# michelebanfi/qLDPC-branched-off

Hardware: AMD Instinct MI355X
Metric: decoded shots/sec, [[144,12,12]] p=0.005 50 BP iters (higher is better)
Workload: dtype f64

## Files before the change

### qldpc-branched-off_amd/csrc/common.h

```cpp
#pragma once
#include <hip/hip_runtime.h>
#include <stdint.h>

#include <algorithm>
#include <cstdarg>
#include <cstdio>
#include <functional>
#include <memory>
#include <mutex>
#include <string>
#include <vector>

#include "../../include/qldpc_hip.h"
#include "stage_layout.h"

#define QLDPC_EXPORT extern "C" __attribute__((visibility("default")))

namespace qldpc {

void set_error(const char *fmt, ...);

#define QLDPC_HIP_TRY(expr)                                                                     \
    do {                                                                                        \
        hipError_t _e = (expr);                                                                 \
// ... 209 lines not shown
    int32_t *d_row_of_slot = nullptr, *d_col_of_slot = nullptr;
    uint8_t *d_deg_of_rslot = nullptr, *d_deg_of_row = nullptr;
    uint16_t *d_deg_of_cslot = nullptr, *d_deg_of_col = nullptr;
    uint16_t *d_ell_col_s = nullptr;
    uint32_t *d_ell_var_s = nullptr;
    int32_t *d_identity = nullptr;
    mutable std::vector<qldpc::DevBuf> owned;
    template <class T> int own(T **view, const std::vector<T> &v) const {
        qldpc::DevBuf b;
        const int rc = qldpc::upload(b, v);
        *view = rc == QLDPC_OK ? b.as<T>() : nullptr;
        if (rc == QLDPC_OK) owned.push_back(std::move(b));
        return rc;
    }
    int32_t *d_regown = nullptr;
    mutable std::mutex mu;
    mutable qldpc::DevBuf ws_msg, ws_qold, ws_vals, ws_misc, ws_queue, ws_list, ws_prior, ws_redo;
    mutable qldpc::DevBuf ws_cs;
    mutable qldpc::DevBuf ws_squeue;
    mutable bool ws_private = false;
    mutable qldpc::StreamHandover ws_hand;
    int ws_acquire(hipStream_t stream) const;
    int ws_release(hipStream_t stream) const;
    mutable std::mutex mu_io;
    mutable qldpc::DevBuf ws_io;
    struct AlphaEntry {
        std::vector<double> host;
        qldpc::PinnedBuf pinned;
        qldpc::DevBuf dev;
        hipEvent_t ready = nullptr;
// ... 15 lines not shown
```

### qldpc-branched-off_amd/csrc/graph.hip

```cpp
#include "common.h"
#include "launchers.h"
#include "regular_plan.h"
#include "regular_own.h"

#include <algorithm>
#include <atomic>
#include <cstring>

namespace qldpc {

static thread_local std::string g_last_error;

void set_error(const char *fmt, ...) {
    char buf[1024];
    va_list ap;
    va_start(ap, fmt);
    vsnprintf(buf, sizeof(buf), fmt, ap);
    va_end(ap);
    g_last_error = buf;
}

int use_device(int device) {
    int count = 0;
    hipError_t e = hipGetDeviceCount(&count);
// ... 291 lines not shown
        }
        std::vector<int32_t> ident(std::max(std::max(m, n), 1));
        for (size_t i = 0; i < ident.size(); i++) ident[i] = (int32_t)i;
        if (rc == QLDPC_OK) rc = g->own(&g->d_row_of_slot, ros);
        if (rc == QLDPC_OK) rc = g->own(&g->d_col_of_slot, cos);
        if (rc == QLDPC_OK) rc = g->own(&g->d_deg_of_rslot, drs);
        if (rc == QLDPC_OK) rc = g->own(&g->d_deg_of_cslot, dcs);
        if (rc == QLDPC_OK) rc = g->own(&g->d_deg_of_row, dr);
        if (rc == QLDPC_OK) rc = g->own(&g->d_deg_of_col, dc);
        if (rc == QLDPC_OK) rc = g->own(&g->d_ell_col_s, ecs);
        if (rc == QLDPC_OK) rc = g->own(&g->d_ell_var_s, evs);
        if (rc == QLDPC_OK) rc = g->own(&g->d_identity, ident);
    }
    if (rc == QLDPC_OK && g->max_row_deg == kRegOwnCdeg && g->max_col_deg == kRegOwnVdeg && n == 2 * m && m <= 1024) {
        std::vector<int32_t> own;
        if (regular_own_assign(m, n, indptr, indices, regular_row_stride(kRegOwnCdeg), own, regular_own_search_choice())) rc = g->own(&g->d_regown, own);
    }
    if (rc != QLDPC_OK) return rc;
    *out = G.release();
    return QLDPC_OK;
}

QLDPC_EXPORT void qldpc_graph_destroy(qldpc_graph *g) {
    if (!g) return;
    (void)hipSetDevice(g->device);
    if (g->wg2_cache) qldpc::wg2_cache_free(g->wg2_cache);
    delete g;
}

QLDPC_EXPORT int qldpc_graph_dims(const qldpc_graph *g, int *m, int *n, int *nnz) {
    QLDPC_REQUIRE(g != nullptr, "graph is NULL");
// ... 6 lines not shown
```

### qldpc-branched-off_amd/csrc/launchers.h

```cpp
#pragma once
#include "common.h"

#include <functional>
#include <vector>

struct qldpc_window_decoder;
struct qldpc_layered_decoder;

namespace qldpc {

struct OsdLaunch;
struct OsdGjArgs;
struct DemTab;
struct SigTab;
struct JudgeSector;
struct EventsSector;

#define QLDPC_FLAG_PUBLIC_MASK 0x0FFFFFFF
#define QLDPC_FLAG_INTERNAL_PRIOR_FINITE 0x40000000
#define QLDPC_FLAG_INTERNAL_PRIOR_LE_CLIP 0x20000000
#define QLDPC_FLAG_INTERNAL_OSD_QUEUE_CLEAN 0x10000000

int minsum_stream_launch(const qldpc_graph *g, int64_t B, const int8_t *d_synd, const double *d_prior, int max_iter,
                         const double *d_alpha, double damping, double clip, int flags, int8_t *d_err, double *d_llr,
// ... 7 lines not shown
int mc_resident_launch(const qldpc_graph *g, int64_t B, const double *d_prior, int max_iter, const double *d_alpha, double clip, int flags,
                       uint64_t seed, int64_t shot_begin, uint32_t thr, int use_osd, const uint64_t *d_Lmask, void *d_cold, hipStream_t stream);
bool regular_supported(const qldpc_graph *g, double clip, int max_iter);
int minsum_regular_launch(const qldpc_graph *g, int64_t B, const int8_t *d_synd, const double *d_prior, int max_iter,
                          const double *d_alpha, double damping, double clip, int flags, bool nanfree, int8_t *d_err, double *d_llr,
                          uint8_t *d_conv, int32_t *d_iter, hipStream_t stream);
int mc_regular_launch(const qldpc_graph *g, int64_t B, const double *d_prior, int max_iter, const double *d_alpha, double clip, int flags,
                      bool nanfree, uint64_t seed, int64_t shot_begin, uint32_t thr, int use_osd, const uint64_t *d_Lmask,
                      void *d_cold, hipStream_t stream, const int32_t *d_shot_list = nullptr, const int32_t *d_shot_count = nullptr);
bool mc_first_table(const qldpc_graph *g, double p0, double alpha0, double clip, int max_iter, unsigned &negbits);
int mc_first_launch(const qldpc_graph *g, int k, const int32_t *d_lptr, const int32_t *d_lidx, int64_t B, uint64_t seed, int64_t shot_begin, uint32_t thr,
                    unsigned negbits, unsigned long long *d_tally, int32_t *d_cont_list, int32_t *d_cont_count, unsigned long long *d_clk, hipStream_t stream);
void mc_first_set_bits(int bits);
void regular_set_list_shots(int s);
void regular_set_own_edges(int v);
int regular_own_search_choice();
void mc_set_big_lanes(int n);
int mc_tail_overlap_choice();
int mc_first_choice();
int mc_regular_fill_cold(void *d_cold, unsigned long long *d_tally, int32_t *d_fail_count, int32_t *d_fail_list, int8_t *f_synd,
                         int8_t *f_err, int8_t *f_hard, double *f_llr, unsigned long long *d_clk);
size_t mc_regular_cold_bytes();
int judge_failed_launch(const qldpc_graph *g, int32_t *d_count, bool reset_counters, int *d_osd_queue, const uint64_t *d_Lmask, const int8_t *f_err, const int8_t *f_synd,
                        const int8_t *f_dec, unsigned long long *d_tally, hipStream_t stream);
bool wave_supported(const qldpc_graph *g, double damping, bool clean);
int wave_kernel_choice();
int minsum_wave_launch(const qldpc_graph *g, int64_t B, const int8_t *d_synd, const double *d_prior, int max_iter, const double *d_alpha,
                       double clip, int flags, int8_t *d_err, double *d_llr, uint8_t *d_conv, int32_t *d_iter, hipStream_t stream);
int mc_wave_launch(const qldpc_graph *g, int64_t B, const double *d_prior, int max_iter, const double *d_alpha, double clip, int flags,
                   uint64_t seed, int64_t shot_begin, uint32_t thr, int use_osd, const uint64_t *d_Lmask, void *d_cold, hipStream_t stream);
// ... 103 lines not shown
```

### qldpc-branched-off_amd/csrc/minsum_regular.hip

```cpp
#include "common.h"
#include "launchers.h"
#include "clocks.h"
#include "mc_common.h"
#include "minsum_common.h"
#include "minsum_f64.h"
#include "regular_plan.h"
#include "regular_own.h"

#include <atomic>
#include <cstdlib>

namespace qldpc {

struct RegArgs {
    int m, n, max_iter, fixed, S, TS;
    const int32_t *indptr, *indices, *colptr, *rowidx, *csc2csr;
    const int32_t *own;
    int64_t B;
    const double *prior, *alpha;
    double damping, clip;
    const int8_t *synd; int8_t *out_err; double *out_llr; uint8_t *out_conv; int32_t *out_iter;
    uint32_t seed_lo, seed_hi, thr; int use_osd;
    int64_t shot_begin;
    const uint64_t *Lmask;
    const int32_t *shot_list, *shot_count;
    const struct RegCold *cold;
    int offV, offE, offL, offI, offA, offT, offD;
};

template <int CDEG, int SKIP = 0>
__device__ __forceinline__ void clean_messages(double (&x)[CDEG], double (&Rprev)[CDEG], bool later, double alpha, double cmin, unsigned synw, double *row) {
    unsigned spw = synw;
#pragma unroll
    for (int k = 0; k < CDEG; k++) {
        if (later) x[k] = x[k] - Rprev[k];
        spw ^= (unsigned)__double2hiint(x[k]);
    }
    double suf[CDEG];
    suf[CDEG - 1] = vmin_abs_u(x[CDEG - 1], cmin);
#pragma unroll
    for (int k = CDEG - 2; k >= 1; k--) suf[k] = vmin_abs(x[k], suf[k + 1]);
    double pre = 0.0;
#pragma unroll
    for (int k = 0; k < CDEG; k++) {
        const double mag = (k == 0) ? suf[1] : (k == CDEG - 1) ? pre : vmin(pre, suf[k + 1]);
        const unsigned sgn = spw ^ (unsigned)__double2hiint(x[k]);
        if (k < CDEG - 1) pre = (k == 0) ? vmin_abs_u(x[0], cmin) : vmin_abs(x[k], pre);
        const double prod = alpha * mag;
        const unsigned hi = ((unsigned)__double2hiint(prod) & 0x7fffffffu) | (sgn & 0x80000000u);
        const double msg = __hiloint2double((int)hi, __double2loint(prod));
        Rprev[k] = msg;
        if (k >= SKIP) row[k - SKIP] = msg;
    }
}

#ifndef QLDPC_LB_T
#define QLDPC_LB_T 512
#define QLDPC_LB_W 8
#endif
template <int CDEG, int VDEG, bool DAMP, bool NANFREE, bool MC, bool FIXED, bool OWN = false>
__global__ __launch_bounds__(QLDPC_LB_T, QLDPC_LB_W) void minsum_regular_kernel(RegArgs A) {
    extern __shared__ unsigned char lds[];
    constexpr int RST = (CDEG % 2 == 0) ? CDEG + 1 : CDEG;
    const int m = A.m, n = A.n, S = A.S, TS = A.TS, max_iter = A.max_iter;
    const int nq = (n + 3) >> 2;
    const int slot = threadIdx.x / TS, member = threadIdx.x - slot * TS;
    const bool in_team = slot < S;
    const int sl = in_team ? slot : 0;
    constexpr bool CLIPMIN = NANFREE && !DAMP;
    constexpr bool ALL = CLIPMIN;
    constexpr bool ZEROFREE = CLIPMIN;
    static_assert(!OWN || (CLIPMIN && CDEG == kRegOwnCdeg && VDEG == kRegOwnVdeg), "edge ownership: the clean (6,3) form");
    constexpr int NOWN = OWN ? kRegOwnOwned : 0;
    double *Dl = reinterpret_cast<double *>(lds + A.offD);
    double *Rl = (ALL && !in_team) ? Dl : reinterpret_cast<double *>(lds) + (size_t)sl * m * RST;
    double *Vl = (ALL && !in_team) ? Dl + RST : reinterpret_cast<double *>(lds + A.offV) + (size_t)sl * n;
    uint32_t *El = reinterpret_cast<uint32_t *>(lds + A.offE) + (size_t)sl * nq;
    unsigned long long *lacc = reinterpret_cast<unsigned long long *>(lds + A.offL) + sl;
    int *I = reinterpret_cast<int *>(lds + A.offI);
    int *unsat = I + 2 * sl;
    int *active = I + 2 * S;
    int *sres = I + 2 * S + 2 + 4 * sl;
    const double *Al = reinterpret_cast<const double *>(lds + A.offA);
    unsigned long long *Tl = reinterpret_cast<unsigned long long *>(lds + A.offT);
    static_assert(CDEG >= 3, "the prefix / suffix chains need a middle edge");
    const double clip = A.clip, nclip = -A.clip, damping = A.damping, one_minus_d = 1.0 - A.damping;
    for (int k = threadIdx.x; k < max_iter; k += blockDim.x) reinterpret_cast<double *>(lds + A.offA)[k] = A.alpha[k];
    if (MC && threadIdx.x < 6) Tl[threadIdx.x] = 0ull;
// ... 28 lines not shown
#pragma unroll
        for (int d = 0; d < VDEG; d++) {
            voff[v][d] = ALL ? d : 0;
            if (OWN) {
                if (has_var[v] && d < 2) voff[v][d] = A.own[member * kRegOwnWords + kRegOwnOffs + 2 * v + d];
                if (has_var[v] && d == 0) vlast[v] = (A.own[member * kRegOwnWords + kRegOwnLast] >> v) & 1;
            } else if (has_var[v]) {
                const int k = A.colptr[j] + d, row = A.rowidx[k];
                voff[v][d] = row * RST + (A.csc2csr[k] - A.indptr[row]);
            }
        }
    }

    auto vcol = [&](int v) { return OWN ? ecol(v) : vj[v]; };

    const int64_t nshots = (MC && A.shot_list) ? (int64_t)*A.shot_count : A.B;
    for (int64_t base = (int64_t)blockIdx.x * S; base < nshots; base += (int64_t)gridDim.x * S) {
        const int64_t b = base + slot;
        const bool valid = in_team && b < nshots;
        bool csyn = false;
        if (MC) {
            if (valid && member < nq) {
                const uint64_t g = (uint64_t)(A.shot_begin + (A.shot_list ? (int64_t)A.shot_list[b] : b));
                uint32_t o[4];
                philox4x32_10((uint32_t)g, (uint32_t)(g >> 32), (uint32_t)member, 0u, A.seed_lo, A.seed_hi, o);
                uint32_t w = 0;
#pragma unroll
                for (int t = 0; t < 4; t++)
                    if (4 * member + t < n && o[t] < A.thr) w |= 1u << (8 * t);
                El[member] = w;
// ... 5 lines not shown
            if (valid && has_check) {
                int s = 0;
#pragma unroll
                for (int k = 0; k < CDEG; k++) s ^= Eb[ecol(k)];
                csyn = s & 1;
                if (csyn) sres[2] = 1;
            }
        } else {
            csyn = (valid && has_check) ? (A.synd[b * m + member] & 1) : false;
        }
        const unsigned synw = csyn ? 0x80000000u : 0u;
        double Rprev[CDEG], Qold[CDEG];
#pragma unroll
        for (int k = 0; k < CDEG; k++) { Rprev[k] = 0.0; Qold[k] = 0.0; }
#pragma unroll
        for (int v = 0; v < 2; v++) if (ALL || has_var[v]) Vl[vj[v]] = vprior[v];
        double Vown[2] = {vprior[0], vprior[1]};
        if (in_team && member == 0) { unsat[0] = 0; unsat[1] = 0; }
        if (threadIdx.x == 0) { const int64_t left = nshots - base; active[0] = (int)(left < S ? left : S); }
        bool done = !valid;
        __syncthreads();

        int it = 0;
        for (; it <= max_iter; it++) {
            const bool in_check = ALL ? (FIXED || !done) : (FIXED ? valid : !done) && has_check;
            double x[CDEG];
            if (in_check) {
                bool par = csyn;
                if (CLIPMIN) {
                    unsigned ph = synw;
#pragma unroll
                    for (int k = 0; k < CDEG; k++) { x[k] = (OWN && k < NOWN) ? Vown[k] : Vl[coff[k]]; ph ^= (unsigned)__double2hiint(x[k]); }
                    par = (int)ph < 0;
                } else {
#pragma unroll
                    for (int k = 0; k < CDEG; k++) { x[k] = Vl[coff[k]]; par ^= (x[k] < 0.0); }
                }
                if (it >= 1 && !done && par) unsat[it & 1] = 1;
            }
            bool skip_msg = false;
            if (!FIXED && it == 1) {
                __syncthreads();
                skip_msg = (unsat[1] == 0);
            }
            if (MC && NANFREE && !DAMP && it == 0) {
                if (in_check && max_iter > 0) {
                    const double p0 = prior0;
                    const bool sneg = csyn != ((((CDEG - 1) & 1) != 0) && (p0 < 0.0));
                    const double mag = Al[0] * fabs(p0);
                    const double msg = sneg ? -mag : mag;
#pragma unroll
                    for (int k = 0; k < CDEG; k++) { Rprev[k] = msg; if (k >= NOWN) Rl[roff + k - NOWN] = msg; }
                }
            } else if (in_check && !skip_msg) {
                if (CLIPMIN && it < max_iter) {
                    clean_messages<CDEG, NOWN>(x, Rprev, it > 0, Al[it], (it > 0) ? clip : INFINITY, synw, Rl + roff);
                } else if (it < max_iter) {
                    const double alpha = Al[it];
                    if (it > 0) {
#pragma unroll
                        for (int k = 0; k < CDEG; k++) {
                            double t = x[k] - Rprev[k];
                            if (!NANFREE) t = (t != t) ? 0.0 : t;
                            t = vmax(vmin(t, clip), nclip);
                            if (DAMP) {
                                const double qd = damping * t + one_minus_d * Qold[k];
                                t = NANFREE ? vmax(vmin(qd, clip), nclip) : clip_only(qd, clip);
                            }
                            if (!NANFREE && !DAMP && ((cnf >> k) & 1u)) t = NAN;
                            x[k] = t;
                        }
// ... 30 lines not shown
                    }
                }
            }
            __syncthreads();
            if (valid && !done) {
                const bool conv = (it >= 1) && (unsat[it & 1] == 0);
                if (conv || it == max_iter) {
                    done = true;
                    if (MC) {
                        const bool exportit = !conv && A.use_osd;
                        if (!exportit) {
                            const uint8_t *Eb = reinterpret_cast<const uint8_t *>(El);
                            unsigned long long lm = 0ull;
#pragma unroll
                            for (int v = 0; v < 2; v++)
                                if (has_var[v] && ((Eb[vcol(v)] ^ ((it >= 1 && Vl[vj[v]] < 0.0) ? 1 : 0)) & 1)) lm ^= A.Lmask[vcol(v)];
                            if (lm) atomicXor(lacc, lm);
                        } else if (member == 0) {
                            active[1] = 1;
                        }
                        if (member == 0) { sres[0] = conv ? 1 : 0; sres[1] = conv ? it - 1 : max_iter - 1; atomicSub(&active[0], 1); }
                    } else {
#pragma unroll
                        for (int v = 0; v < 2; v++)
                            if (has_var[v]) {
                                const double xo = (it >= 1) ? Vl[vj[v]] : 0.0;
                                A.out_llr[b * n + vcol(v)] = xo;
                                A.out_err[b * n + vcol(v)] = (xo < 0.0) ? 1 : 0;
                            }
                        if (member == 0) {
                            A.out_conv[b] = conv ? 1 : 0;
                            A.out_iter[b] = conv ? it - 1 : max_iter - 1;
                            atomicSub(&active[0], 1);
                        }
                    }
                }
            }
            if (in_team && member == 0) unsat[(it + 1) & 1] = 0;
            if (it < max_iter && (ALL ? (FIXED || !done) : (FIXED ? valid : !done))) {
#pragma unroll
                for (int v = 0; v < 2; v++)
                    if (ALL || has_var[v]) {
                        double s = 0.0;
                        if (OWN) {
                            const double o1 = Rl[voff[v][0]], o2 = Rl[voff[v][1]], own = Rprev[v];
                            s = ZEROFREE ? o1 : s + o1;
                            s += vlast[v] ? o2 : own; s += vlast[v] ? own : o2;
                        } else {
#pragma unroll
                            for (int d = 0; d < VDEG; d++) s = (ZEROFREE && d == 0) ? Rl[voff[v][0]] : s + Rl[voff[v][d]];
                        }
                        const double xv = s + vprior[v];
                        Vl[vj[v]] = xv;
                        Vown[v] = xv;
                    }
            }
            __syncthreads();
            if ((!FIXED || ALL) && active[0] == 0) { it++; break; }
        }
        if (ALL && FIXED) {
            unsigned parity = 0u;
            const __attribute__((address_space(4))) double *alpha_tab = (const __attribute__((address_space(4))) double *)A.alpha;
            double alpha_it = (it < max_iter) ? Al[it] : 0.0;
            for (; it < max_iter; it++) {
                double x[CDEG];
                unsigned ph = synw;
#pragma unroll
                for (int k = 0; k < CDEG; k++) x[k] = (OWN && k < NOWN) ? Vown[k] : Vl[coff[k]];
#pragma unroll
                for (int k = 0; k < CDEG; k++) ph ^= (unsigned)__double2hiint(x[k]);
                parity |= ph;
                clean_messages<CDEG, NOWN>(x, Rprev, true, alpha_it, clip, synw, Rl + roff);
                __syncthreads();
                __builtin_amdgcn_s_setprio(1);
                double r[2][VDEG];
#pragma unroll
                for (int v = 0; v < 2; v++)
#pragma unroll
                    for (int d = 0; d < VDEG - (OWN ? 1 : 0); d++) r[v][d] = Rl[voff[v][d]];
#pragma unroll
                for (int v = 0; v < 2; v++) {
                    if (OWN) {
                        const double o2 = r[v][1], own = Rprev[v];
                        r[v][1] = vlast[v] ? o2 : own;
                        r[v][2] = vlast[v] ? own : o2;
                    }
                    double s = 0.0;
#pragma unroll
                    for (int d = 0; d < VDEG; d++) s = (ZEROFREE && d == 0) ? r[v][0] : s + r[v][d];
                    Vown[v] = s + vprior[v];
                    Vl[vj[v]] = Vown[v];
                }
                __builtin_amdgcn_s_setprio(0);
                alpha_it = alpha_tab[it + 1 < max_iter ? it + 1 : max_iter - 1];
                __syncthreads();
            }
            if (it == max_iter) {
                unsigned ph = synw;
#pragma unroll
                for (int k = 0; k < CDEG; k++) ph ^= (unsigned)__double2hiint(Vl[coff[k]]);
                parity |= ph;
            }
            reinterpret_cast<unsigned *>(Dl + RST + 2)[0] = parity;
        }
        __syncthreads();
        if (MC) {
            if (active[1]) {
                const RegCold C = *A.cold;
                if (valid && member == 0 && sres[0] == 0 && A.use_osd) {
                    const int f = atomicAdd(C.fail_count, 1);
                    sres[3] = f;
                    C.fail_list[f] = f;
                }
                __syncthreads();
                const int f = valid ? sres[3] : -1;
                if (f >= 0) {
                    const uint8_t *Eb = reinterpret_cast<const uint8_t *>(El);
                    if (has_check) C.f_synd[(int64_t)f * m + member] = csyn ? 1 : 0;
#pragma unroll
                    for (int v = 0; v < 2; v++)
                        if (has_var[v]) {
                            const double xo = (max_iter >= 1) ? Vl[vj[v]] : 0.0;
                            C.f_llr[(int64_t)f * n + vcol(v)] = xo;
                            C.f_hard[(int64_t)f * n + vcol(v)] = (xo < 0.0) ? 1 : 0;
                            C.f_err[(int64_t)f * n + vcol(v)] = (int8_t)Eb[vcol(v)];
                        }
                }
                __syncthreads();
            }
            if ((int)threadIdx.x < S && base + threadIdx.x < nshots) {
                const int *r = I + 2 * S + 2 + 4 * threadIdx.x;
                const unsigned long long lm = *(reinterpret_cast<unsigned long long *>(lds + A.offL) + threadIdx.x);
                const bool exported = (r[0] == 0) && A.use_osd;
                atomicAdd(&Tl[0], 1ull);
                if (r[0]) atomicAdd(&Tl[2], 1ull);
                atomicAdd(&Tl[3], (unsigned long long)(r[1] + 1));
                if (!r[2]) atomicAdd(&Tl[4], 1ull);
// ... 62 lines not shown
    return plan_regular_shape(cdeg, vdeg, g->m, g->n, max_iter, QLDPC_LB_T, force_S, P);
}

bool regular_supported(const qldpc_graph *g, double clip, int max_iter) {
    RegPlan P;
    return clip >= 0.0 && plan_regular(g, max_iter, P);
}

template <int CDEG, int VDEG, bool MC, bool FIXED>
static int launch_reg2(const RegArgs &A, bool damp, bool nanfree, unsigned grid, unsigned block, size_t lds, hipStream_t stream) {
    if (damp) {
        if (MC) return QLDPC_ERR_UNSUPPORTED;
        hipLaunchKernelGGL((minsum_regular_kernel<CDEG, VDEG, true, false, false, FIXED>), dim3(grid), dim3(block), lds, stream, A);
    } else if (nanfree && A.clip > 0.0) {
        if constexpr (CDEG == kRegOwnCdeg && VDEG == kRegOwnVdeg) {
            if (A.own) {
                hipLaunchKernelGGL((minsum_regular_kernel<CDEG, VDEG, false, true, MC, FIXED, true>), dim3(grid), dim3(block), lds, stream, A);
                QLDPC_HIP_TRY(hipGetLastError());
                return QLDPC_OK;
            }
        }
        hipLaunchKernelGGL((minsum_regular_kernel<CDEG, VDEG, false, true, MC, FIXED>), dim3(grid), dim3(block), lds, stream, A);
    } else {
        hipLaunchKernelGGL((minsum_regular_kernel<CDEG, VDEG, false, false, MC, FIXED>), dim3(grid), dim3(block), lds, stream, A);
    }
    QLDPC_HIP_TRY(hipGetLastError());
    return QLDPC_OK;
}

template <int CDEG, int VDEG, bool MC>
static int launch_reg(const RegArgs &A, bool damp, bool nanfree, unsigned grid, unsigned block, size_t lds, hipStream_t stream) {
// ... 7 lines not shown
    if (P.cdeg == 4) return launch_reg<4, 2, MC>(A, damp, nanfree, grid, P.block, P.lds, stream);
    return launch_reg<8, 4, MC>(A, damp, nanfree, grid, P.block, P.lds, stream);
}

static void fill_common(const qldpc_graph *g, const RegPlan &P, RegArgs &A, int64_t B, const double *d_prior, int max_iter,
                        const double *d_alpha, double damping, double clip, int flags) {
    A = RegArgs{};
    A.m = g->m; A.n = g->n; A.max_iter = max_iter; A.fixed = (flags & QLDPC_FLAG_FIXED_ITERS) ? 1 : 0;
    A.S = P.S; A.TS = P.TS;
    A.indptr = g->d_indptr; A.indices = g->d_indices; A.colptr = g->d_colptr; A.rowidx = g->d_rowidx; A.csc2csr = g->d_csc2csr;
    A.own = (g_own_edges.load() && P.cdeg == kRegOwnCdeg) ? g->d_regown : nullptr;
    A.B = B; A.prior = d_prior; A.alpha = d_alpha; A.damping = damping; A.clip = clip;
    A.offV = P.offV; A.offE = P.offE; A.offL = P.offL; A.offI = P.offI; A.offA = P.offA; A.offT = P.offT; A.offD = P.offD;
}

static unsigned persistent_grid(int64_t B, int S) {
    const int64_t groups = (B + S - 1) / S;
    const int64_t cap = 256 * 12;
    return (unsigned)(groups < cap ? (groups > 0 ? groups : 1) : cap);
}

int minsum_regular_launch(const qldpc_graph *g, int64_t B, const int8_t *d_synd, const double *d_prior, int max_iter,
                          const double *d_alpha, double damping, double clip, int flags, bool nanfree, int8_t *d_err, double *d_llr,
                          uint8_t *d_conv, int32_t *d_iter, hipStream_t stream) {
    RegPlan P;
    if (!plan_regular(g, max_iter, P)) { set_error("graph is not regular (6,3)/(4,2)/(8,4)"); return QLDPC_ERR_UNSUPPORTED; }
    RegArgs A;
    fill_common(g, P, A, B, d_prior, max_iter, d_alpha, damping, clip, flags);
    A.synd = d_synd; A.out_err = d_err; A.out_llr = d_llr; A.out_conv = d_conv; A.out_iter = d_iter;
    return dispatch_reg<false>(P, A, damping != 1.0, nanfree, persistent_grid(B, P.S), stream);
}

int mc_regular_launch(const qldpc_graph *g, int64_t B, const double *d_prior, int max_iter, const double *d_alpha, double clip, int flags,
                      bool nanfree, uint64_t seed, int64_t shot_begin, uint32_t thr, int use_osd, const uint64_t *d_Lmask,
                      void *d_cold, hipStream_t stream, const int32_t *d_shot_list, const int32_t *d_shot_count) {
    RegPlan P;
    if (!plan_regular(g, max_iter, P, d_shot_list ? g_list_shots : 0)) { set_error("graph is not regular (6,3)/(4,2)/(8,4)"); return QLDPC_ERR_UNSUPPORTED; }
    RegArgs A;
    fill_common(g, P, A, B, d_prior, max_iter, d_alpha, 1.0, clip, flags);
    A.seed_lo = (uint32_t)seed; A.seed_hi = (uint32_t)(seed >> 32); A.thr = thr; A.use_osd = use_osd; A.shot_begin = shot_begin;
    A.Lmask = d_Lmask; A.cold = reinterpret_cast<const RegCold *>(d_cold);
    A.shot_list = d_shot_list; A.shot_count = d_shot_count;
    const unsigned grid = d_shot_list ? persistent_grid(std::max<int64_t>(B / 16, 1), P.S) * (unsigned)(g_list_shots > 0 ? 4 : 1) : persistent_grid(B, P.S);
    return dispatch_reg<true>(P, A, false, nanfree, grid, stream);
}

int mc_regular_fill_cold(void *d_cold, unsigned long long *d_tally, int32_t *d_fail_count, int32_t *d_fail_list, int8_t *f_synd,
                         int8_t *f_err, int8_t *f_hard, double *f_llr, unsigned long long *d_clk) {
    RegCold C{d_tally, d_fail_count, d_fail_list, f_synd, f_err, f_hard, f_llr, d_clk};
    QLDPC_HIP_TRY(hipMemcpy(d_cold, &C, sizeof(C), hipMemcpyHostToDevice));
    return QLDPC_OK;
}
size_t mc_regular_cold_bytes() { return sizeof(RegCold); }

// ... 10 lines not shown
```

### qldpc-branched-off_amd/csrc/options.hip

```cpp
#include "common.h"
#include "launchers.h"

#include <atomic>
#include <cstring>

namespace qldpc {

static std::atomic<int> g_opt_kernel{0}, g_opt_first{1}, g_opt_tail{1}, g_opt_presort{-1}, g_opt_own_search{1};
int regular_own_search_choice() { return g_opt_own_search.load(); }
int osd_presort_choice() { return g_opt_presort.load(); }
int wave_kernel_choice() { return g_opt_kernel.load(); }
int mc_first_choice() { return g_opt_first.load(); }
int mc_tail_overlap_choice() { return g_opt_tail.load(); }
#ifdef QLDPC_EXPERIMENTS
extern std::atomic<int> g_opt_wave_cpl, g_opt_wave_rst, g_opt_wave_grid;
#endif

}

QLDPC_EXPORT int qldpc_set_option(const char *name, int value) {
    QLDPC_REQUIRE(name != nullptr, "name is NULL");
    if (!std::strcmp(name, "mc_first_iteration")) { QLDPC_REQUIRE(value == 0 || value == 1, "mc_first_iteration: 0 or 1"); qldpc::g_opt_first = value; return QLDPC_OK; }
    if (!std::strcmp(name, "mc_tail_overlap")) { QLDPC_REQUIRE(value >= 0 && value <= 2, "mc_tail_overlap: 0, 1 or 2"); qldpc::g_opt_tail = value; return QLDPC_OK; }
    if (!std::strcmp(name, "mc_first_bits")) { QLDPC_REQUIRE(value == 8 || value == 16 || value == 32, "mc_first_bits: 8, 16 or 32"); qldpc::mc_first_set_bits(value); return QLDPC_OK; }
    if (!std::strcmp(name, "osd_presort")) { QLDPC_REQUIRE(value >= -1 && value <= 65535, "osd_presort: -1 .. 65535"); qldpc::g_opt_presort = value; return QLDPC_OK; }
    if (!std::strcmp(name, "mc_big_lanes")) { QLDPC_REQUIRE(value >= 2 && value <= 8, "mc_big_lanes: 2 .. 8"); qldpc::mc_set_big_lanes(value); return QLDPC_OK; }
    if (!std::strcmp(name, "mc_list_shots")) { QLDPC_REQUIRE(value >= 0 && value <= 16, "mc_list_shots: 0 .. 16"); qldpc::regular_set_list_shots(value); return QLDPC_OK; }
    if (!std::strcmp(name, "regular_own_search")) { QLDPC_REQUIRE(value == 0 || value == 1, "regular_own_search: 0 or 1"); qldpc::g_opt_own_search = value; return QLDPC_OK; }
    if (!std::strcmp(name, "regular_own_edges")) { QLDPC_REQUIRE(value == 0 || value == 1, "regular_own_edges: 0 or 1"); qldpc::regular_set_own_edges(value); return QLDPC_OK; }
    const bool wave_opt =!std::strcmp(name, "regular_kernel") || !std::strcmp(name, "wave_cpl") || !std::strcmp(name, "wave_rst") || !std::strcmp(name, "wave_grid");
#ifdef QLDPC_EXPERIMENTS
    if (!std::strcmp(name, "regular_kernel")) { QLDPC_REQUIRE(value >= 0 && value <= 2, "regular_kernel: 0, 1 or 2"); qldpc::g_opt_kernel = value; return QLDPC_OK; }
    if (!std::strcmp(name, "wave_cpl")) { QLDPC_REQUIRE(value == 0 || value == 4 || value == 5 || value == 6 || value == 9, "wave_cpl: 0, 4, 5, 6 or 9"); qldpc::g_opt_wave_cpl = value; return QLDPC_OK; }
    if (!std::strcmp(name, "wave_rst")) { QLDPC_REQUIRE(value == 0 || value == 6 || value == 7, "wave_rst: 0, 6 or 7"); qldpc::g_opt_wave_rst = value; return QLDPC_OK; }
    if (!std::strcmp(name, "wave_grid")) { QLDPC_REQUIRE(value >= 0 && value <= 32, "wave_grid: 0 .. 32"); qldpc::g_opt_wave_grid = value; return QLDPC_OK; }
#else
    if (wave_opt) {
        if (value == 0) return QLDPC_OK;
        qldpc::set_error("option '%s': the wave-private kernel is a measured-and-rejected experiment (libqldpc_hip_experiments.so, make experiments)", name);
        return QLDPC_ERR_UNSUPPORTED;
    }
#endif
    (void)wave_opt;
    qldpc::set_error("unknown option '%s'", name);
// ... 25 lines not shown
```

Measured before the change: 131.5 million.

## Place regular min-sum LDS messages and posteriors by edge-coloured bank-conflict-free layout

Adds a host-built per-thread placement table that remaps every LDS address used for check-to-variable messages and variable posteriors in the owned-edge (6,3) fixed-iteration kernel. Addresses come from a bipartite edge colouring with Kempe-chain local search, so the gathers and stores of each wavefront are spread across LDS banks. The aim is to remove LDS bank conflicts in the inner BP loop. In exchange each thread loads a 64-byte record at kernel start, holds extra index registers, and the graph handle caches host-side tables.

```diff
diff --git a/qldpc-branched-off_amd/csrc/common.h b/qldpc-branched-off_amd/csrc/common.h
--- a/qldpc-branched-off_amd/csrc/common.h
+++ b/qldpc-branched-off_amd/csrc/common.h
@@ -247,6 +247,10 @@
         return rc;
     }
     int32_t *d_regown = nullptr;
+    std::vector<int32_t> regown;
+    struct PlaceEntry { int S = 0, block = 0, placed = 0, offD = 0; qldpc::DevBuf dev; };
+    mutable std::mutex mu_place;
+    mutable std::vector<PlaceEntry> place_cache;
     mutable std::mutex mu;
     mutable qldpc::DevBuf ws_msg, ws_qold, ws_vals, ws_misc, ws_queue, ws_list, ws_prior, ws_redo;
     mutable qldpc::DevBuf ws_cs;
diff --git a/qldpc-branched-off_amd/csrc/graph.hip b/qldpc-branched-off_amd/csrc/graph.hip
--- a/qldpc-branched-off_amd/csrc/graph.hip
+++ b/qldpc-branched-off_amd/csrc/graph.hip
@@ -329,7 +329,7 @@
     }
     if (rc == QLDPC_OK && g->max_row_deg == kRegOwnCdeg && g->max_col_deg == kRegOwnVdeg && n == 2 * m && m <= 1024) {
         std::vector<int32_t> own;
-        if (regular_own_assign(m, n, indptr, indices, regular_row_stride(kRegOwnCdeg), own, regular_own_search_choice())) rc = g->own(&g->d_regown, own);
+        if (regular_own_assign(m, n, indptr, indices, regular_row_stride(kRegOwnCdeg), own, regular_own_search_choice())) { rc = g->own(&g->d_regown, own); g->regown = std::move(own); }
     }
     if (rc != QLDPC_OK) return rc;
     *out = G.release();
diff --git a/qldpc-branched-off_amd/csrc/launchers.h b/qldpc-branched-off_amd/csrc/launchers.h
--- a/qldpc-branched-off_amd/csrc/launchers.h
+++ b/qldpc-branched-off_amd/csrc/launchers.h
@@ -45,6 +45,7 @@
 void mc_first_set_bits(int bits);
 void regular_set_list_shots(int s);
 void regular_set_own_edges(int v);
+void regular_set_place(int v);
 int regular_own_search_choice();
 void mc_set_big_lanes(int n);
 int mc_tail_overlap_choice();
diff --git a/qldpc-branched-off_amd/csrc/minsum_regular.hip b/qldpc-branched-off_amd/csrc/minsum_regular.hip
--- a/qldpc-branched-off_amd/csrc/minsum_regular.hip
+++ b/qldpc-branched-off_amd/csrc/minsum_regular.hip
@@ -6,6 +6,7 @@
 #include "minsum_f64.h"
 #include "regular_plan.h"
 #include "regular_own.h"
+#include "regular_place.h"
 
 #include <atomic>
 #include <cstdlib>
@@ -16,6 +17,7 @@
     int m, n, max_iter, fixed, S, TS;
     const int32_t *indptr, *indices, *colptr, *rowidx, *csc2csr;
     const int32_t *own;
+    const int32_t *place;
     int64_t B;
     const double *prior, *alpha;
     double damping, clip;
@@ -29,7 +31,8 @@
 };
 
 template <int CDEG, int SKIP = 0>
-__device__ __forceinline__ void clean_messages(double (&x)[CDEG], double (&Rprev)[CDEG], bool later, double alpha, double cmin, unsigned synw, double *row) {
+__device__ __forceinline__ void clean_messages(double (&x)[CDEG], double (&Rprev)[CDEG], bool later, double alpha, double cmin, unsigned synw, double *row,
+                                               const int *at = nullptr) {
     unsigned spw = synw;
 #pragma unroll
     for (int k = 0; k < CDEG; k++) {
@@ -50,7 +53,7 @@
         const unsigned hi = ((unsigned)__double2hiint(prod) & 0x7fffffffu) | (sgn & 0x80000000u);
         const double msg = __hiloint2double((int)hi, __double2loint(prod));
         Rprev[k] = msg;
-        if (k >= SKIP) row[k - SKIP] = msg;
+        if (k >= SKIP) row[at ? at[k - SKIP] : k - SKIP] = msg;
     }
 }
 
@@ -72,6 +75,7 @@
     constexpr bool ZEROFREE = CLIPMIN;
     static_assert(!OWN || (CLIPMIN && CDEG == kRegOwnCdeg && VDEG == kRegOwnVdeg), "edge ownership: the clean (6,3) form");
     constexpr int NOWN = OWN ? kRegOwnOwned : 0;
+    constexpr bool PLACE = OWN && FIXED;
     double *Dl = reinterpret_cast<double *>(lds + A.offD);
     double *Rl = (ALL && !in_team) ? Dl : reinterpret_cast<double *>(lds) + (size_t)sl * m * RST;
     double *Vl = (ALL && !in_team) ? Dl + RST : reinterpret_cast<double *>(lds + A.offV) + (size_t)sl * n;
@@ -130,6 +134,28 @@
 
     auto vcol = [&](int v) { return OWN ? ecol(v) : vj[v]; };
 
+    double *Lb = reinterpret_cast<double *>(lds);
+    int pgat[CDEG], mgat[4], msto[4];
+#pragma unroll
+    for (int k = 0; k < CDEG; k++) pgat[k] = 0;
+#pragma unroll
+    for (int k = 0; k < 4; k++) { mgat[k] = 0; msto[k] = 0; }
+    if (PLACE) {
+        static_assert(kRegPlaceWords == 16, "a record is four 16-byte loads");
+        const int4 *rec4 = reinterpret_cast<const int4 *>(A.place) + (size_t)threadIdx.x * 4;
+        const int4 r0 = rec4[0], r1 = rec4[1], r2 = rec4[2], r3 = rec4[3];
+        const int pr[kRegPlaceWords] = {r0.x, r0.y, r0.z, r0.w, r1.x, r1.y, r1.z, r1.w, r2.x, r2.y, r2.z, r2.w, r3.x, r3.y, r3.z, r3.w};
+#pragma unroll
+        for (int k = 0; k < CDEG; k++) pgat[k] = (k < NOWN) ? pr[kRegPlacePostStore + k] : pr[kRegPlacePostGather + k - NOWN];
+#pragma unroll
+        for (int k = 0; k < 4; k++) { mgat[k] = pr[kRegPlaceMsgGather + k]; msto[k] = pr[kRegPlaceMsgStore + k]; }
+    }
+    auto Vof = [&](int k) -> double & { return PLACE ? Lb[pgat[k]] : Vl[coff[k]]; };
+    auto Vmine = [&](int v) -> double & { return PLACE ? Lb[pgat[v]] : Vl[vj[v]]; };
+    auto Rin = [&](int v, int d) -> double & { return PLACE ? Lb[mgat[2 * v + d]] : Rl[voff[v][d]]; };
+    double *const rowp = PLACE ? Lb : Rl + roff;
+    const int *const rowat = PLACE ? msto : nullptr;
+
     const int64_t nshots = (MC && A.shot_list) ? (int64_t)*A.shot_count : A.B;
     for (int64_t base = (int64_t)blockIdx.x * S; base < nshots; base += (int64_t)gridDim.x * S) {
         const int64_t b = base + slot;
@@ -165,7 +191,7 @@
 #pragma unroll
         for (int k = 0; k < CDEG; k++) { Rprev[k] = 0.0; Qold[k] = 0.0; }
 #pragma unroll
-        for (int v = 0; v < 2; v++) if (ALL || has_var[v]) Vl[vj[v]] = vprior[v];
+        for (int v = 0; v < 2; v++) if (ALL || has_var[v]) Vmine(v) = vprior[v];
         double Vown[2] = {vprior[0], vprior[1]};
         if (in_team && member == 0) { unsat[0] = 0; unsat[1] = 0; }
         if (threadIdx.x == 0) { const int64_t left = nshots - base; active[0] = (int)(left < S ? left : S); }
@@ -181,7 +207,7 @@
                 if (CLIPMIN) {
                     unsigned ph = synw;
 #pragma unroll
-                    for (int k = 0; k < CDEG; k++) { x[k] = (OWN && k < NOWN) ? Vown[k] : Vl[coff[k]]; ph ^= (unsigned)__double2hiint(x[k]); }
+                    for (int k = 0; k < CDEG; k++) { x[k] = (OWN && k < NOWN) ? Vown[k] : Vof(k); ph ^= (unsigned)__double2hiint(x[k]); }
                     par = (int)ph < 0;
                 } else {
 #pragma unroll
@@ -201,11 +227,11 @@
                     const double mag = Al[0] * fabs(p0);
                     const double msg = sneg ? -mag : mag;
 #pragma unroll
-                    for (int k = 0; k < CDEG; k++) { Rprev[k] = msg; if (k >= NOWN) Rl[roff + k - NOWN] = msg; }
+                    for (int k = 0; k < CDEG; k++) { Rprev[k] = msg; if (k >= NOWN) rowp[PLACE ? msto[k - NOWN] : k - NOWN] = msg; }
                 }
             } else if (in_check && !skip_msg) {
                 if (CLIPMIN && it < max_iter) {
-                    clean_messages<CDEG, NOWN>(x, Rprev, it > 0, Al[it], (it > 0) ? clip : INFINITY, synw, Rl + roff);
+                    clean_messages<CDEG, NOWN>(x, Rprev, it > 0, Al[it], (it > 0) ? clip : INFINITY, synw, rowp, rowat);
                 } else if (it < max_iter) {
                     const double alpha = Al[it];
                     if (it > 0) {
@@ -266,7 +292,7 @@
                             unsigned long long lm = 0ull;
 #pragma unroll
                             for (int v = 0; v < 2; v++)
-                                if (has_var[v] && ((Eb[vcol(v)] ^ ((it >= 1 && Vl[vj[v]] < 0.0) ? 1 : 0)) & 1)) lm ^= A.Lmask[vcol(v)];
+                                if (has_var[v] && ((Eb[vcol(v)] ^ ((it >= 1 && Vmine(v) < 0.0) ? 1 : 0)) & 1)) lm ^= A.Lmask[vcol(v)];
                             if (lm) atomicXor(lacc, lm);
                         } else if (member == 0) {
                             active[1] = 1;
@@ -276,7 +302,7 @@
 #pragma unroll
                         for (int v = 0; v < 2; v++)
                             if (has_var[v]) {
-                                const double xo = (it >= 1) ? Vl[vj[v]] : 0.0;
+                                const double xo = (it >= 1) ? Vmine(v) : 0.0;
                                 A.out_llr[b * n + vcol(v)] = xo;
                                 A.out_err[b * n + vcol(v)] = (xo < 0.0) ? 1 : 0;
                             }
@@ -295,7 +321,7 @@
                     if (ALL || has_var[v]) {
                         double s = 0.0;
                         if (OWN) {
-                            const double o1 = Rl[voff[v][0]], o2 = Rl[voff[v][1]], own = Rprev[v];
+                            const double o1 = Rin(v, 0), o2 = Rin(v, 1), own = Rprev[v];
                             s = ZEROFREE ? o1 : s + o1;
                             s += vlast[v] ? o2 : own; s += vlast[v] ? own : o2;
                         } else {
@@ -303,7 +329,7 @@
                             for (int d = 0; d < VDEG; d++) s = (ZEROFREE && d == 0) ? Rl[voff[v][0]] : s + Rl[voff[v][d]];
                         }
                         const double xv = s + vprior[v];
-                        Vl[vj[v]] = xv;
+                        Vmine(v) = xv;
                         Vown[v] = xv;
                     }
             }
@@ -318,18 +344,18 @@
                 double x[CDEG];
                 unsigned ph = synw;
 #pragma unroll
-                for (int k = 0; k < CDEG; k++) x[k] = (OWN && k < NOWN) ? Vown[k] : Vl[coff[k]];
+                for (int k = 0; k < CDEG; k++) x[k] = (OWN && k < NOWN) ? Vown[k] : Vof(k);
 #pragma unroll
                 for (int k = 0; k < CDEG; k++) ph ^= (unsigned)__double2hiint(x[k]);
                 parity |= ph;
-                clean_messages<CDEG, NOWN>(x, Rprev, true, alpha_it, clip, synw, Rl + roff);
+                clean_messages<CDEG, NOWN>(x, Rprev, true, alpha_it, clip, synw, rowp, rowat);
                 __syncthreads();
                 __builtin_amdgcn_s_setprio(1);
                 double r[2][VDEG];
 #pragma unroll
                 for (int v = 0; v < 2; v++)
 #pragma unroll
-                    for (int d = 0; d < VDEG - (OWN ? 1 : 0); d++) r[v][d] = Rl[voff[v][d]];
+                    for (int d = 0; d < VDEG - (OWN ? 1 : 0); d++) r[v][d] = Rin(v, d);
 #pragma unroll
                 for (int v = 0; v < 2; v++) {
                     if (OWN) {
@@ -341,7 +367,7 @@
 #pragma unroll
                     for (int d = 0; d < VDEG; d++) s = (ZEROFREE && d == 0) ? r[v][0] : s + r[v][d];
                     Vown[v] = s + vprior[v];
-                    Vl[vj[v]] = Vown[v];
+                    Vmine(v) = Vown[v];
                 }
                 __builtin_amdgcn_s_setprio(0);
                 alpha_it = alpha_tab[it + 1 < max_iter ? it + 1 : max_iter - 1];
@@ -350,7 +376,7 @@
             if (it == max_iter) {
                 unsigned ph = synw;
 #pragma unroll
-                for (int k = 0; k < CDEG; k++) ph ^= (unsigned)__double2hiint(Vl[coff[k]]);
+                for (int k = 0; k < CDEG; k++) ph ^= (unsigned)__double2hiint(Vof(k));
                 parity |= ph;
             }
             reinterpret_cast<unsigned *>(Dl + RST + 2)[0] = parity;
@@ -372,7 +398,7 @@
 #pragma unroll
                     for (int v = 0; v < 2; v++)
                         if (has_var[v]) {
-                            const double xo = (max_iter >= 1) ? Vl[vj[v]] : 0.0;
+                            const double xo = (max_iter >= 1) ? Vmine(v) : 0.0;
                             C.f_llr[(int64_t)f * n + vcol(v)] = xo;
                             C.f_hard[(int64_t)f * n + vcol(v)] = (xo < 0.0) ? 1 : 0;
                             C.f_err[(int64_t)f * n + vcol(v)] = (int8_t)Eb[vcol(v)];
@@ -465,7 +491,7 @@
         hipLaunchKernelGGL((minsum_regular_kernel<CDEG, VDEG, true, false, false, FIXED>), dim3(grid), dim3(block), lds, stream, A);
     } else if (nanfree && A.clip > 0.0) {
         if constexpr (CDEG == kRegOwnCdeg && VDEG == kRegOwnVdeg) {
-            if (A.own) {
+            if (A.own && (A.place || !FIXED)) {
                 hipLaunchKernelGGL((minsum_regular_kernel<CDEG, VDEG, false, true, MC, FIXED, true>), dim3(grid), dim3(block), lds, stream, A);
                 QLDPC_HIP_TRY(hipGetLastError());
                 return QLDPC_OK;
@@ -503,6 +529,43 @@
     A.offV = P.offV; A.offE = P.offE; A.offL = P.offL; A.offI = P.offI; A.offA = P.offA; A.offT = P.offT; A.offD = P.offD;
 }
 
+static std::atomic<int> g_place{1};
+void regular_set_place(int v) { g_place = v; }
+
+static int regular_place_table(const qldpc_graph *g, const RegPlan &P, const int32_t **out) {
+    *out = nullptr;
+    if (g->regown.size() != (size_t)g->m * kRegOwnWords) { set_error("regular min-sum: the graph handle has no ownership table"); return QLDPC_ERR_INVALID; }
+    const int rst = regular_row_stride(kRegOwnCdeg);
+    std::lock_guard<std::mutex> lk(g->mu_place);
+    auto find = [&](int placed, int offD) -> const qldpc_graph::PlaceEntry * {
+        for (const auto &e : g->place_cache) if (e.S == P.S && e.block == (int)P.block && e.placed == placed && e.offD == offD) return &e;
+        return nullptr;
+    };
+    auto add = [&](int placed, int offD, const std::vector<int32_t> &rec) -> int {
+        qldpc_graph::PlaceEntry e;
+        e.S = P.S; e.block = (int)P.block; e.placed = placed; e.offD = offD;
+        if (!rec.empty()) { const int rc = upload(e.dev, rec); if (rc != QLDPC_OK) return rc; }
+        g->place_cache.push_back(std::move(e));
+        return QLDPC_OK;
+    };
+    std::vector<int32_t> rec;
+    if (g_place.load()) {
+        if (!find(1, 0)) {
+            regular_place_build(g->m, g->regown.data(), P, rst, rec);
+            const int rc = add(1, 0, rec);
+            if (rc != QLDPC_OK) return rc;
+        }
+        if (const auto *e = find(1, 0); e && e->dev.p) { *out = e->dev.as<int32_t>(); return QLDPC_OK; }
+    }
+    if (!find(0, P.offD)) {
+        regular_place_linear(g->m, g->regown.data(), P, rst, rec);
+        const int rc = add(0, P.offD, rec);
+        if (rc != QLDPC_OK) return rc;
+    }
+    *out = find(0, P.offD)->dev.as<int32_t>();
+    return QLDPC_OK;
+}
+
 static unsigned persistent_grid(int64_t B, int S) {
     const int64_t groups = (B + S - 1) / S;
     const int64_t cap = 256 * 12;
@@ -516,6 +579,7 @@
     if (!plan_regular(g, max_iter, P)) { set_error("graph is not regular (6,3)/(4,2)/(8,4)"); return QLDPC_ERR_UNSUPPORTED; }
     RegArgs A;
     fill_common(g, P, A, B, d_prior, max_iter, d_alpha, damping, clip, flags);
+    if (A.own && A.fixed && damping == 1.0 && nanfree && clip > 0.0) { const int rc = regular_place_table(g, P, &A.place); if (rc != QLDPC_OK) return rc; }
     A.synd = d_synd; A.out_err = d_err; A.out_llr = d_llr; A.out_conv = d_conv; A.out_iter = d_iter;
     return dispatch_reg<false>(P, A, damping != 1.0, nanfree, persistent_grid(B, P.S), stream);
 }
@@ -527,6 +591,7 @@
     if (!plan_regular(g, max_iter, P, d_shot_list ? g_list_shots : 0)) { set_error("graph is not regular (6,3)/(4,2)/(8,4)"); return QLDPC_ERR_UNSUPPORTED; }
     RegArgs A;
     fill_common(g, P, A, B, d_prior, max_iter, d_alpha, 1.0, clip, flags);
+    if (A.own && A.fixed && nanfree && clip > 0.0) { const int rc = regular_place_table(g, P, &A.place); if (rc != QLDPC_OK) return rc; }
     A.seed_lo = (uint32_t)seed; A.seed_hi = (uint32_t)(seed >> 32); A.thr = thr; A.use_osd = use_osd; A.shot_begin = shot_begin;
     A.Lmask = d_Lmask; A.cold = reinterpret_cast<const RegCold *>(d_cold);
     A.shot_list = d_shot_list; A.shot_count = d_shot_count;
diff --git a/qldpc-branched-off_amd/csrc/options.hip b/qldpc-branched-off_amd/csrc/options.hip
--- a/qldpc-branched-off_amd/csrc/options.hip
+++ b/qldpc-branched-off_amd/csrc/options.hip
@@ -28,6 +28,7 @@
     if (!std::strcmp(name, "mc_list_shots")) { QLDPC_REQUIRE(value >= 0 && value <= 16, "mc_list_shots: 0 .. 16"); qldpc::regular_set_list_shots(value); return QLDPC_OK; }
     if (!std::strcmp(name, "regular_own_search")) { QLDPC_REQUIRE(value == 0 || value == 1, "regular_own_search: 0 or 1"); qldpc::g_opt_own_search = value; return QLDPC_OK; }
     if (!std::strcmp(name, "regular_own_edges")) { QLDPC_REQUIRE(value == 0 || value == 1, "regular_own_edges: 0 or 1"); qldpc::regular_set_own_edges(value); return QLDPC_OK; }
+    if (!std::strcmp(name, "regular_place")) { QLDPC_REQUIRE(value == 0 || value == 1, "regular_place: 0 or 1"); qldpc::regular_set_place(value); return QLDPC_OK; }
     const bool wave_opt =!std::strcmp(name, "regular_kernel") || !std::strcmp(name, "wave_cpl") || !std::strcmp(name, "wave_rst") || !std::strcmp(name, "wave_grid");
 #ifdef QLDPC_EXPERIMENTS
     if (!std::strcmp(name, "regular_kernel")) { QLDPC_REQUIRE(value >= 0 && value <= 2, "regular_kernel: 0, 1 or 2"); qldpc::g_opt_kernel = value; return QLDPC_OK; }
diff --git a/qldpc-branched-off_amd/csrc/regular_place.h b/qldpc-branched-off_amd/csrc/regular_place.h
--- /dev/null
+++ b/qldpc-branched-off_amd/csrc/regular_place.h
@@ -0,0 +1,266 @@
+#pragma once
+#include <algorithm>
+#include <cstdint>
+#include <utility>
+#include <vector>
+
+#include "regular_own.h"
+
+namespace qldpc {
+
+static const int kRegPlaceWords = 16;
+static const int kRegPlacePostGather = 0, kRegPlaceMsgGather = 4, kRegPlacePostStore = 8, kRegPlaceMsgStore = 10, kRegPlaceEdges = 14;
+static const int kRegPlaceStreams = 14;
+static const int kRegPlaceStored = kRegOwnCdeg - kRegOwnOwned;
+static const int kRegPlaceKempeMoves = 8000;
+#ifndef QLDPC_PLACE_THRESHOLD
+#define QLDPC_PLACE_THRESHOLD 4
+#endif
+static const int kRegPlaceThreshold = QLDPC_PLACE_THRESHOLD;
+
+struct RegPlaceCost {
+    long long gather = 0, post_store = 0, msg_store = 0, post_store_over6 = 0, msg_store_over6 = 0, stream[kRegPlaceStreams] = {};
+};
+
+inline RegPlaceCost regular_place_cost(const int32_t *rec, int block) {
+    RegPlaceCost C;
+    auto group_cost = [&](int word, int t0, int lanes) {
+        int addr[32], worst = 0;
+        for (int l = 0; l < lanes; l++) addr[l] = rec[(size_t)(t0 + l) * kRegPlaceWords + word];
+        std::sort(addr, addr + lanes);
+        int load[32] = {};
+        for (int l = 0; l < lanes; l++) {
+            if (l && addr[l] == addr[l - 1]) continue;
+            const int c = ++load[addr[l] & (lanes - 1)];
+            if (c > worst) worst = c;
+        }
+        return worst;
+    };
+    for (int w = 0; w < kRegPlaceStreams; w++) {
+        const bool store = w >= kRegPlacePostStore;
+        for (int t0 = 0; t0 < block; t0 += 64) {
+            int cyc = 0;
+            if (!store) cyc = group_cost(w, t0, 32) + group_cost(w, t0 + 32, 32);
+            else for (int g = 0; g < 4; g++) cyc += group_cost(w, t0 + 16 * g, 16);
+            C.stream[w] += cyc;
+            if (!store) C.gather += cyc;
+            else if (w < kRegPlaceMsgStore) { C.post_store += cyc; C.post_store_over6 += std::max(0, cyc - 6); }
+            else { C.msg_store += cyc; C.msg_store_over6 += std::max(0, cyc - 6); }
+        }
+    }
+    return C;
+}
+
+inline void regular_place_linear(int m, const int32_t *own, const RegPlan &P, int rst, std::vector<int32_t> &rec) {
+    const int n = 2 * m, vbase = P.offV / 8, dbase = P.offD / 8;
+    rec.assign((size_t)P.block * kRegPlaceWords, 0);
+    for (int t = 0; t < (int)P.block; t++) {
+        int32_t *r = &rec[(size_t)t * kRegPlaceWords];
+        const int s = t / P.TS, i = t - s * P.TS;
+        if (s < P.S && i < m) {
+            const int32_t *o = own + (size_t)i * kRegOwnWords;
+            for (int k = 0; k < kRegPlaceStored; k++) {
+                r[kRegPlacePostGather + k] = vbase + s * n + o[kRegOwnGather + k];
+                r[kRegPlaceMsgGather + k] = s * m * rst + o[kRegOwnOffs + k];
+                r[kRegPlaceMsgStore + k] = (s * m + i) * rst + k;
+                r[kRegPlaceEdges] |= (kRegOwnOwned + k) << (4 * k);
+            }
+            for (int v = 0; v < kRegOwnOwned; v++) r[kRegPlacePostStore + v] = vbase + s * n + i + v * m;
+        } else {
+            for (int k = 0; k < kRegPlaceStored; k++) {
+                r[kRegPlacePostGather + k] = dbase + rst + (k & 1);
+                r[kRegPlaceMsgGather + k] = dbase + (k & 1);
+                r[kRegPlaceMsgStore + k] = dbase + k;
+            }
+            for (int v = 0; v < kRegOwnOwned; v++) r[kRegPlacePostStore + v] = dbase + rst + v;
+        }
+    }
+}
+
+struct RegPlaceColouring {
+    int D = 0;
+    std::vector<std::pair<int, int>> edges;
+    std::vector<int> col, at_l, at_r;
+    bool colour(int nl, int nr, int colours) {
+        D = colours;
+        col.assign(edges.size(), -1); at_l.assign((size_t)nl * D, -1); at_r.assign((size_t)nr * D, -1);
+        std::vector<int> path;
+        for (int e = 0; e < (int)edges.size(); e++) {
+            const int u = edges[e].first, v = edges[e].second;
+            int a = -1, b = -1;
+            for (int c = 0; c < D && a < 0; c++) if (at_l[(size_t)u * D + c] < 0) a = c;
+            for (int c = 0; c < D && b < 0; c++) if (at_r[(size_t)v * D + c] < 0) b = c;
+            if (a < 0 || b < 0) return false;
+            if (at_r[(size_t)v * D + a] >= 0) {
+                path.clear();
+                for (int x = at_r[(size_t)v * D + a], want = b; x >= 0; want = (want == a) ? b : a) {
+                    path.push_back(x);
+                    x = (want == b) ? at_l[(size_t)edges[x].first * D + b] : at_r[(size_t)edges[x].second * D + a];
+                }
+                flip(path, a, b);
+            }
+            set(e, a);
+        }
+        return true;
+    }
+    void set(int e, int c) { col[e] = c; at_l[(size_t)edges[e].first * D + c] = e; at_r[(size_t)edges[e].second * D + c] = e; }
+    void flip(const std::vector<int> &comp, int a, int b) {
+        for (int x : comp) { at_l[(size_t)edges[x].first * D + col[x]] = -1; at_r[(size_t)edges[x].second * D + col[x]] = -1; }
+        for (int x : comp) set(x, col[x] == a ? b : a);
+    }
+    void component(int e, int a, int b, std::vector<int> &comp, std::vector<int> &mark, int stamp) const {
+        comp.clear(); comp.push_back(e); mark[e] = stamp;
+        for (size_t at = 0; at < comp.size(); at++) {
+            const int x = comp[at], o = (col[x] == a) ? b : a;
+            for (int y : {at_l[(size_t)edges[x].first * D + o], at_r[(size_t)edges[x].second * D + o]})
+                if (y >= 0 && mark[y] != stamp) { mark[y] = stamp; comp.push_back(y); }
+        }
+    }
+    bool proper() const {
+        for (size_t e = 0; e < edges.size(); e++)
+            if (col[e] < 0 || col[e] >= D || at_l[(size_t)edges[e].first * D + col[e]] != (int)e || at_r[(size_t)edges[e].second * D + col[e]] != (int)e) return false;
+        return true;
+    }
+};
+
+inline bool regular_place_build(int m, const int32_t *own, const RegPlan &P, int rst, std::vector<int32_t> &rec, int moves = kRegPlaceKempeMoves) {
+    rec.clear();
+    const int n = 2 * m, S = P.S, block = (int)P.block;
+    if (m <= 0 || S <= 0 || P.TS != m || block % 64 || block < S * m || rst < kRegPlaceStored) return false;
+    const int nwin = block / 32, n16 = block / 16, msg_words = 4 * block, post_base = msg_words, post_words = 2 * block;
+    if ((long long)(msg_words + post_words) * 8 > (long long)P.offV + (long long)S * n * 8) return false;
+    auto lane = [&](int s, int i) { return s * m + i; };
+
+    std::vector<int> rd_check((size_t)n * 2, -1), rd_edge((size_t)n * 2, -1);
+    for (int i = 0; i < m; i++)
+        for (int q = 0; q < kRegPlaceStored; q++) {
+            const int g = own[(size_t)i * kRegOwnWords + kRegOwnGather + q];
+            if (g < 0 || g >= n || g % m == i) return false;
+            const int at = rd_check[(size_t)g * 2] < 0 ? 0 : 1;
+            if (rd_check[(size_t)g * 2 + at] >= 0) return false;
+            rd_check[(size_t)g * 2 + at] = i; rd_edge[(size_t)g * 2 + at] = q;
+        }
+    for (int g = 0; g < n; g++) if (rd_check[(size_t)g * 2 + 1] < 0 || rd_check[(size_t)g * 2] == rd_check[(size_t)g * 2 + 1]) return false;
+    std::vector<int> tail(n, -1), next_q(m, 0);
+    {
+        auto unused_at = [&](int i) {
+            for (int &q = next_q[i]; q < kRegPlaceStored; q++) {
+                const int g = own[(size_t)i * kRegOwnWords + kRegOwnGather + q];
+                if (tail[g] < 0) return g;
+            }
+            return -1;
+        };
+        for (int start = 0; start < m; start++)
+            for (int u = start, g; (g = unused_at(u)) >= 0;) {
+                const int at = rd_check[(size_t)g * 2] == u ? 0 : 1;
+                tail[g] = at;
+                u = rd_check[(size_t)g * 2 + 1 - at];
+            }
+    }
+    std::vector<int> pos((size_t)m * kRegPlaceStored, -1), ntail(m, 0), nhead(m, 0);
+    for (int g = 0; g < n; g++) {
+        const int at = tail[g], u = rd_check[(size_t)g * 2 + at], w = rd_check[(size_t)g * 2 + 1 - at];
+        if (ntail[u] >= 2 || nhead[w] >= 2) return false;
+        pos[(size_t)u * kRegPlaceStored + rd_edge[(size_t)g * 2 + at]] = ntail[u]++;
+        pos[(size_t)w * kRegPlaceStored + rd_edge[(size_t)g * 2 + 1 - at]] = 2 + nhead[w]++;
+    }
+    for (int x : pos) if (x < 0) return false;
+
+    rec.assign((size_t)block * kRegPlaceWords, 0);
+    auto word = [&](int t, int w) -> int32_t & { return rec[(size_t)t * kRegPlaceWords + w]; };
+    for (int s = 0; s < S; s++)
+        for (int i = 0; i < m; i++)
+            for (int q = 0; q < kRegPlaceStored; q++) word(lane(s, i), kRegPlaceEdges) |= (kRegOwnOwned + q) << (4 * pos[(size_t)i * kRegPlaceStored + q]);
+
+    {
+        RegPlaceColouring K;
+        struct Item { int tail_lane, tail_k, head_lane, head_k, store_lane, v; };
+        std::vector<Item> items;
+        for (int s = 0; s < S; s++)
+            for (int g = 0; g < n; g++) {
+                const int at = tail[g], u = rd_check[(size_t)g * 2 + at], w = rd_check[(size_t)g * 2 + 1 - at];
+                items.push_back({lane(s, u), pos[(size_t)u * kRegPlaceStored + rd_edge[(size_t)g * 2 + at]], lane(s, w),
+                                 pos[(size_t)w * kRegPlaceStored + rd_edge[(size_t)g * 2 + 1 - at]] - 2, lane(s, g % m), g / m});
+            }
+        for (int t = S * m; t < block; t++)
+            for (int v = 0; v < kRegOwnOwned; v++) items.push_back({t, v, t, v, t, v});
+        for (const Item &it : items) K.edges.emplace_back(it.tail_k * nwin + it.tail_lane / 32, it.head_k * nwin + it.head_lane / 32);
+        if (!K.colour(2 * nwin, 2 * nwin, 32)) { rec.clear(); return false; }
+        const int ni = (int)items.size();
+        std::vector<int> grp(ni), cnt((size_t)2 * n16 * 16, 0), comp, mark(ni, -1), bad;
+        for (int e = 0; e < ni; e++) { grp[e] = items[e].v * n16 + items[e].store_lane / 16; cnt[(size_t)grp[e] * 16 + (K.col[e] & 15)]++; }
+        auto score = [&]() {
+            long long tot = 0, over = 0;
+            for (int w = 0; w < 2 * n16; w += 4) {
+                int cyc = 0;
+                for (int g = w; g < w + 4; g++) cyc += *std::max_element(&cnt[(size_t)g * 16], &cnt[(size_t)g * 16] + 16);
+                tot += cyc; over += std::max(0, cyc - 6);
+            }
+            return over * 100000 + tot;
+        };
+        auto recount = [&](const std::vector<int> &c, int d) { for (int x : c) cnt[(size_t)grp[x] * 16 + (K.col[x] & 15)] += d; };
+        uint64_t state = 0x9e3779b97f4a7c15ull;
+        auto rnd = [&](uint32_t below) {
+            uint64_t z = (state += 0x9e3779b97f4a7c15ull);
+            z = (z ^ (z >> 30)) * 0xbf58476d1ce4e5b9ull; z = (z ^ (z >> 27)) * 0x94d049bb133111ebull; z ^= z >> 31;
+            return (uint32_t)(((z >> 32) * below) >> 32);
+        };
+        long long cur = score(), best = cur;
+        RegPlaceColouring best_K = K;
+        for (int mv = 0; mv < moves; mv++) {
+            bad.clear();
+            for (int e = 0; e < ni; e++) if (cnt[(size_t)grp[e] * 16 + (K.col[e] & 15)] > 1) bad.push_back(e);
+            if (bad.empty()) break;
+            const int e = bad[rnd((uint32_t)bad.size())], a = K.col[e];
+            int free_c[32], nfree = 0;
+            for (int c = 0; c < 32; c++) if (c != a && cnt[(size_t)grp[e] * 16 + (c & 15)] == 0) free_c[nfree++] = c;
+            const int b = nfree ? free_c[rnd((uint32_t)nfree)] : (a + 1 + (int)rnd(31)) & 31;
+            K.component(e, a, b, comp, mark, mv);
+            recount(comp, -1); K.flip(comp, a, b); recount(comp, +1);
+            const long long now = score();
+            if (now <= cur + (long long)kRegPlaceThreshold * (moves - mv) / moves) {
+                cur = now;
+                if (cur < best) { best = cur; best_K = K; }
+            } else { recount(comp, -1); K.flip(comp, a, b); recount(comp, +1); }
+        }
+        if (best < cur) K = best_K;
+        if (!K.proper()) { rec.clear(); return false; }
+        std::vector<int> rank(32, 0);
+        for (int e = 0; e < ni; e++) {
+            const int c = K.col[e], a = post_base + 32 * rank[c]++ + c;
+            if (a >= post_base + post_words) { rec.clear(); return false; }
+            const Item &it = items[e];
+            word(it.tail_lane, kRegPlacePostGather + it.tail_k) = a;
+            word(it.head_lane, kRegPlacePostGather + 2 + it.head_k) = a;
+            word(it.store_lane, kRegPlacePostStore + it.v) = a;
+        }
+    }
+
+    {
+        RegPlaceColouring K;
+        struct Item { int read_lane, stream, store_lane, t; };
+        std::vector<Item> items;
+        for (int s = 0; s < S; s++)
+            for (int i = 0; i < m; i++)
+                for (int vd = 0; vd < 4; vd++) {
+                    const int off = own[(size_t)i * kRegOwnWords + kRegOwnOffs + vd], r = off / rst, q = off - r * rst;
+                    if (off < 0 || r >= m || q >= kRegPlaceStored) { rec.clear(); return false; }
+                    items.push_back({lane(s, i), vd, lane(s, r), pos[(size_t)r * kRegPlaceStored + q]});
+                }
+        for (int t = S * m; t < block; t++)
+            for (int k = 0; k < 4; k++) items.push_back({t, k, t, k});
+        for (const Item &it : items) K.edges.emplace_back(it.stream * n16 + it.read_lane / 16, it.t * n16 + it.store_lane / 16);
+        if (!K.colour(4 * n16, 4 * n16, 16) || !K.proper()) { rec.clear(); return false; }
+        std::vector<int> rank(32, 0);
+        for (int e = 0; e < (int)items.size(); e++) {
+            const Item &it = items[e];
+            const int bank = K.col[e] + 16 * ((it.read_lane / 16) & 1), a = 32 * rank[bank]++ + bank;
+            if (a >= msg_words) { rec.clear(); return false; }
+            word(it.read_lane, kRegPlaceMsgGather + it.stream) = a;
+            word(it.store_lane, kRegPlaceMsgStore + it.t) = a;
+        }
+    }
+    return true;
+}
+
+}
```

Measured after the change: 140.1 million (median of 6 runs). +6.6%, better.
